# VolkmannB/bayesian-inference-with-explicit-and-implicit-prior-knowledge

Measured on AMD Instinct MI355X. Metric: particle-steps/sec (N x (T-1) / wall), SingleMassOscillator PGAS conditional-SMC sweep, higher is better.
Workload: dtype f64; 1 GPU; SingleMassOscillator PGAS sweep, nx=2, M=41 Hilbert basis (BASELINE.json configs[1]), N=1048576 particles/GPU, T=2000, fp64; particles_per_gpu=1048576, particles_total=1048576, T=2000, partition=single GPU, launch=every sweep enqueued launch by launch, verified=not checked in this run (--full checks the last timed sweep's traces), parallelism=1 GPU

## Files before the change

### bayesian-inference-with-explicit-and-implicit-prior-knowledge_amd/csrc/pgas_api.hip

```cpp
#include <hip/hip_runtime.h>
#include <hip/hip_ext.h>
#include <dlfcn.h>
#include <rccl/rccl.h>

#include <algorithm>
#include <cmath>
#include <cstdio>
#include <cstdlib>
#include <cstring>
#include <string>
#include <vector>

#include "../../include/pgas_hip.h"
#include "pgas_kernels.hip.h"
#include "pgas_resample.hip.h"
#include "pgas_suffstats.hip.h"
#include "pgas_marginal.hip.h"
#include "pgas_marginal_runs.hip.h"
#include "pgas_chains.hip.h"
#include "../../include/pgas_marginal.h"

#ifndef PG_W3
#define PG_W3 2
#endif
// ... 570 lines not shown
    hipLaunchKernelGGL(c->basis, dim3((unsigned)((np + PG_BLK - 1) / PG_BLK)), dim3(PG_BLK), 0, (hipStream_t)stream, c->md, c->d_idx, x_dev, np, t, phi_dev);
    KCHK(c, "k_basis_eval");
    return PGAS_OK;
}

int pgas_aux_states(pgas_ctx* c, const double* x_dev, int32_t t, double* aux_dev, void* stream) {
    if (!c) return PGAS_E_ARG;
    if (!x_dev || !aux_dev || t < 0 || t >= c->md.T) FAIL(c, PGAS_E_ARG, "pgas_aux_states: bad argument");
    if (!c->have_params) FAIL(c, PGAS_E_STATE, "pgas_aux_states: call pgas_set_params first");
    DeviceGuard guard(c->device);
    hipLaunchKernelGGL(c->var.aux, dim3(c->md.nseg), dim3(PG_BLK), 0, (hipStream_t)stream, c->md, (const TransParams*)c->d_tp, t, x_dev, aux_dev);
    KCHK(c, "k_aux");
    return PGAS_OK;
}

int pgas_init_state(pgas_ctx* c, uint64_t seed, const double* ref0_host, double* x0_dev, void* stream) {
    if (!c) return PGAS_E_ARG;
    if (!ref0_host || !x0_dev) FAIL(c, PGAS_E_ARG, "pgas_init_state: NULL argument");
    DeviceGuard guard(c->device);
    hipStream_t st = (hipStream_t)stream;
    HIPCHK(c, hipMemcpyAsync(c->d_ref, ref0_host, c->md.nx * sizeof(double), hipMemcpyHostToDevice, st));
    hipLaunchKernelGGL(c->init, dim3((c->md.N + PG_BLK - 1) / PG_BLK), dim3(PG_BLK), 0, st, c->md, seed, (const SweepParams*)nullptr, c->d_m0L0, c->d_ref, x0_dev);
    KCHK(c, "k_init");
    return PGAS_OK;
}

static Peers peers_for(const pgas_ctx* c, int parity) {
    Peers p = c->peers;
    for (int r = 0; r < p.world; ++r) {
        p.c1[r] = c->peer_c1[parity][r];
        p.c2[r] = c->peer_c2[parity][r];
    }
    return p;
}

static void install_own_peers(pgas_ctx* c) {
    const int r = c->rank;
    for (int k = 0; k < PG_RB_NKIND; ++k) c->peer_blk[r][k].assign(c->rs[k].blk.begin(), c->rs[k].blk.end());
    c->bt_dirty = true;
    for (int i = 0; i < 2; ++i) {
        c->peer_c1[i][r] = c->sb[i].c1;
        c->peer_c2[i][r] = c->sb[i].c2;
    }
}

static const char* peer_row(const pgas_ctx* c, int r, int kind, int t) {
    const RowStore& s = c->rs[kind];
    return c->peer_blk[r][kind][(size_t)t >> s.shift] + (size_t)(t & ((1 << s.shift) - 1)) * s.row_bytes;
}

static int upload_bt_table(pgas_ctx* c, hipStream_t st, BtTab* out) {
    const int nb = std::max(c->rs[PG_RB_X].nblk, c->rs[PG_RB_ANC].nblk);
    const size_t entries = (size_t)c->world * 2 * nb;
    if (c->bt_dirty || c->d_bt_entries != entries) {
        std::vector<const void*> h(entries, nullptr);
        for (int r = 0; r < c->world; ++r) {
            const auto& bx = c->peer_blk[r][PG_RB_X];
            const auto& ba = c->peer_blk[r][PG_RB_ANC];
            for (size_t b = 0; b < bx.size(); ++b) h[((size_t)r * 2) * nb + b] = bx[b];
            for (size_t b = 0; b < ba.size(); ++b) h[((size_t)r * 2 + 1) * nb + b] = ba[b];
        }
        HIPCHK(c, hipStreamSynchronize(st));
        if (c->d_bt_entries != entries) {
            hipFree(c->d_bt);
            c->d_bt = nullptr; c->d_bt_entries = 0;
            HIPCHK(c, hipMalloc(&c->d_bt, entries * sizeof(void*)));
            c->d_bt_entries = entries;
        }
        HIPCHK(c, hipMemcpy(c->d_bt, h.data(), entries * sizeof(void*), hipMemcpyHostToDevice));
        c->bt_dirty = false;
    }
    out->blk = c->d_bt;
    out->nblk_max = nb;
    out->shift_x = c->rs[PG_RB_X].shift;
    out->shift_anc = c->rs[PG_RB_ANC].shift;
    out->entries = (int32_t)entries;
    return PGAS_OK;
}

static int launch_backtrace(pgas_ctx* c, const UpperHdr* hdr, double* traj_dev, hipStream_t st) {
    BtTab tab;
    int rc = upload_bt_table(c, st, &tab);
    if (rc) return rc;
    const size_t lds = tab.entries <= 2048 ? (size_t)tab.entries * sizeof(void*) : 0;
    hipLaunchKernelGGL(k_backtrace, dim3(1), dim3(64), lds, st, c->md.N, c->md.T, c->md.nx, tab, c->world, hdr, traj_dev);
    KCHK(c, "k_backtrace");
    return PGAS_OK;
}

static int launch_groups(pgas_ctx* c, const ScanBufs& sb, int ncdf, hipStream_t st) {
    const int n1 = (c->md.nseg_g + PG_GRP - 1) / PG_GRP;
    hipLaunchKernelGGL(k_groups, dim3((n1 * ncdf + 3) / 4), dim3(256), 0, st, c->md.nseg_g, ncdf, sb);
    KCHK(c, "k_groups");
    return PGAS_OK;
}

static int launch_count(pgas_ctx* c, const ScanBufs& sb, int parity, int what, double u, hipStream_t st) {
    hipLaunchKernelGGL(k_count, dim3(1), dim3(PG_BLK), 0, st, c->md.Ng, c->md.nseg_g, sb, peers_for(c, parity), what, u, what == 1 ? (const SweepParams*)c->d_sp : (const SweepParams*)nullptr);
    KCHK(c, "k_count");
    return PGAS_OK;
}

static bool sweep_is_local(const pgas_ctx* c) { return c->local_groups && c->world == 1 && !c->sharded && c->md.nseg_g <= PG_LOCAL_NSEG && !c->force_slow; }

static bool sweep_tail_groups(const pgas_ctx* c) { return !c->sharded && c->world == 1 && c->tail_groups; }

static int launch_step(pgas_ctx* c, int t, bool local, hipStream_t st, hipEvent_t e0, hipEvent_t e1) {
    const DevModel& md = c->md;
    const int N = md.N, T = md.T;
    StepArgs ar;
    ar.t = t;
    ar.mode = (t < T ? PG_RS_SCAN : 0) | (t > 1 ? PG_RS_SEARCH : 0);
    ar.sp = c->d_sp;
    ar.u_res = c->d_ures;
    ar.u_anc = c->d_uanc;
    ar.la_t = t < T ? (const double*)c->rs[PG_RB_LA].row(t) : (const double*)nullptr;
    ar.h_t = t < T ? (const double*)c->rs[PG_RB_H].row(t) : (const double*)nullptr;
    ar.ln_prev = (const double*)c->rs[PG_RB_LN].row(t - 1);
    ar.anc_in = AncIn{};
    ar.anc_in.has_prev = t > 2 ? 1 : 0;
    if (t > 1)
        for (int r = 0; r < c->world; ++r) {
            ar.anc_in.la_s[r] = (const double*)peer_row(c, r, PG_RB_LA, t - 1);
            ar.anc_in.h_s[r] = (const double*)peer_row(c, r, PG_RB_H, t - 1);
            if (t > 2) {
                ar.anc_in.ln_p[r] = (const double*)peer_row(c, r, PG_RB_LN, t - 2);
                ar.anc_in.la_p[r] = (const double*)peer_row(c, r, PG_RB_LA, t - 2);
                ar.anc_in.anc_p[r] = (const int32_t*)peer_row(c, r, PG_RB_ANC, t - 3);
            }
        }
    ar.anc_out = t > 1 ? (int32_t*)c->rs[PG_RB_ANC].row(t - 2) : (int32_t*)nullptr;
    ar.logw_out = t == T ? c->logw_last : ((c->logw_trace && t > 1) ? c->logw_trace + (size_t)(t - 1) * N : (double*)nullptr);
    const ScanBufs& sp = c->sb[(t - 1) & 1];
    const ScanBufs& sn = c->sb[t & 1];
    const Peers pr = peers_for(c, (t - 1) & 1);
    auto kern = local ? k_step<PG_WM_LOCAL, false> : (sweep_tail_groups(c) ? k_step<PG_WM_GROUPS, true> : k_step<PG_WM_GROUPS, false>);
    if (e0 || e1) hipExtLaunchKernelGGL(kern, dim3(md.nseg + 1), dim3(PG_BLK), 0, st, e0, e1, 0, md, ar, sp, sn, pr);
    else hipLaunchKernelGGL(kern, dim3(md.nseg + 1), dim3(PG_BLK), 0, st, md, ar, sp, sn, pr);
    KCHK(c, "k_step");
    return PGAS_OK;
}

int pgas_step(pgas_ctx* c, int32_t t, uint64_t seed, const double* logw_dev, const double* x_dev, const double* ref_t_host,
              double* logw_new_dev, double* x_new_dev, int32_t* anc_dev, void* stream) {
    if (!c) return PGAS_E_ARG;
    if (!x_dev || !ref_t_host || !logw_new_dev || !x_new_dev || !anc_dev) FAIL(c, PGAS_E_ARG, "pgas_step: NULL argument");
    if (t < 0 || t >= c->md.T) FAIL(c, PGAS_E_ARG, "pgas_step: t = %d outside [0, %d)", t, c->md.T);
    if (!c->have_params) FAIL(c, PGAS_E_STATE, "pgas_step: call pgas_set_params first");
    if (c->sharded) FAIL(c, PGAS_E_STATE, "pgas_step: not available on a shard context");
    DeviceGuard guard(c->device);
    hipStream_t st = (hipStream_t)stream;
    const DevModel& md = c->md;
    install_own_peers(c);
    HIPCHK(c, hipMemcpyAsync(c->d_ref, ref_t_host, md.nx * sizeof(double), hipMemcpyHostToDevice, st));
    if (c->corrected && !c->aux_buf) HIPCHK(c, hipMalloc(&c->aux_buf, (size_t)md.N * md.nx * sizeof(double)));
    hipLaunchKernelGGL(c->var.front, dim3(md.nseg), dim3(PG_BLK), 0, st, md, (const TransParams*)c->d_tp, t, seed, x_dev, logw_dev, c->d_ref, c->corrected,
                       c->corrected ? c->aux_buf : x_new_dev, c->sb[0]);
    KCHK(c, "k_front");
    int rc = launch_groups(c, c->sb[0], 2, st);
    if (rc) return rc;
    rc = launch_count(c, c->sb[0], 0, 0, pgas_rng_uniform(seed, PGAS_STREAM_ANCESTOR, (uint32_t)t), st);
    if (rc) return rc;
    const Peers pr = peers_for(c, 0);
    if (c->corrected) {
        hipLaunchKernelGGL(c->back_corrected, dim3(md.nseg), dim3(PG_BLK), 0, st, md, (const TransParams*)c->d_tp, t, seed,
                           pgas_rng_uniform(seed, PGAS_STREAM_RESAMPLE, (uint32_t)t), c->aux_buf, c->d_ref, c->sb[0], pr, anc_dev, x_new_dev, logw_new_dev);
    } else {
        hipLaunchKernelGGL(c->back, dim3(md.nseg), dim3(PG_BLK), 0, st, md, t,
// ... 493 lines not shown
    }
    FAIL(c, PGAS_E_ARG, "pgas_set_option: unknown option %d", option);
}

int pgas_get_profile(pgas_ctx* c, int64_t* launches, double* total_ms, int64_t* propagate_launches, double* propagate_ms, void* stream) {
    if (!c) return PGAS_E_ARG;
    if (!launches || !total_ms || !propagate_launches || !propagate_ms) FAIL(c, PGAS_E_ARG, "pgas_get_profile: NULL argument");
    DeviceGuard guard(c->device);
    HIPCHK(c, hipStreamSynchronize((hipStream_t)stream));
    double sum = 0.0;
    for (int i = 0; i + 1 < c->ev_used; i += 2) {
        float ms = 0.f;
        HIPCHK(c, hipEventElapsedTime(&ms, c->ev[i], c->ev[i + 1]));
        sum += ms;
    }
    *launches = c->ev_used / 2;
    *total_ms = sum;
    double psum = 0.0;
    for (int i = 0; i + 1 < c->evp_used; i += 2) {
        float ms = 0.f;
        HIPCHK(c, hipEventElapsedTime(&ms, c->evp[i], c->evp[i + 1]));
        psum += ms;
    }
    *propagate_launches = c->evp_used / 2;
    *propagate_ms = psum;
    return PGAS_OK;
}

int pgas_get_launch_info(pgas_ctx* c, int32_t* info4) {
    if (!c) return PGAS_E_ARG;
    if (!info4) FAIL(c, PGAS_E_ARG, "pgas_get_launch_info: NULL argument");
    info4[0] = c->last_chunk;
    info4[1] = (c->last_small ? 3 : (sweep_is_local(c) ? 1 : (sweep_tail_groups(c) ? 2 : 0))) + (c->last_graph ? 16 : 0) + ((c->d_mxi && c->use_mx && !c->last_small) ? 32 : 0);
    info4[2] = c->md.JP;
    info4[3] = c->var_P;
    return PGAS_OK;
}

#ifdef PG_DEBUG_DUMP
int pgas_debug_dump(double* out ) {
    return hipMemcpyFromSymbol(out, HIP_SYMBOL(g_dbg), sizeof(double) * 4 * 64) == hipSuccess ? 0 : -2;
}
#endif
#ifdef PG_STAMPS
int pgas_debug_stamps(unsigned long long* out ) {
    return hipMemcpyFromSymbol(out, HIP_SYMBOL(g_stamps), sizeof(unsigned long long) * 2048 * 16) == hipSuccess ? 0 : -2;
}
#endif


static int systematic_impl(pgas_ctx* c, double u, const double* u_dev, const double* logw_dev, int32_t* idx_dev, void* stream) {
    if (c->sharded) FAIL(c, PGAS_E_STATE, "pgas_systematic_resample: not available on a shard context");
    DeviceGuard guard(c->device);
    hipStream_t st = (hipStream_t)stream;
    const DevModel& md = c->md;
    install_own_peers(c);
    hipLaunchKernelGGL(k_segscan, dim3(md.nseg), dim3(PG_BLK), 0, st, md.N, logw_dev, c->sb[0]);
    KCHK(c, "k_segscan");
    int rc = launch_groups(c, c->sb[0], 1, st);
    if (rc) return rc;
    hipLaunchKernelGGL(k_systematic, dim3(md.nseg), dim3(PG_BLK), 0, st, md, u, u_dev, c->sb[0], peers_for(c, 0), idx_dev);
    KCHK(c, "k_systematic");
    return PGAS_OK;
}

int pgas_systematic_resample(pgas_ctx* c, double u, const double* logw_dev, int32_t* idx_dev, void* stream) {
    if (!c) return PGAS_E_ARG;
    if (!logw_dev || !idx_dev || !(u >= 0.0 && u < 1.0)) FAIL(c, PGAS_E_ARG, "pgas_systematic_resample: bad argument");
    return systematic_impl(c, u, nullptr, logw_dev, idx_dev, stream);
}

int pgas_systematic_resample_dev(pgas_ctx* c, const double* u_dev, const double* logw_dev, int32_t* idx_dev, void* stream) {
    if (!c) return PGAS_E_ARG;
    if (!u_dev || !logw_dev || !idx_dev) FAIL(c, PGAS_E_ARG, "pgas_systematic_resample_dev: NULL argument");
    return systematic_impl(c, 0.0, u_dev, logw_dev, idx_dev, stream);
}

int pgas_reconstruct_trajectory(pgas_ctx* c, const double* x_dev, const int32_t* anc_dev, int32_t T, int32_t nx, int64_t idx,
                                double* traj_dev, void* stream) {
    if (!c) return PGAS_E_ARG;
    if (!x_dev || !traj_dev || T < 1 || nx < 1 || idx < 0 || idx >= c->md.N || (T > 1 && !anc_dev))
        FAIL(c, PGAS_E_ARG, "pgas_reconstruct_trajectory: bad argument");
    DeviceGuard guard(c->device);
    hipLaunchKernelGGL(k_backtrace_idx, dim3(1), dim3(64), 0, (hipStream_t)stream, c->md.N, T, nx, x_dev, anc_dev, idx, traj_dev);
    KCHK(c, "k_backtrace_idx");
    return PGAS_OK;
}

int pgas_shard_setup(pgas_ctx* c, int32_t rank, int32_t world) {
    if (!c) return PGAS_E_ARG;
    if (world < 1 || world > PG_MAX_RANKS || rank < 0 || rank >= world) FAIL(c, PGAS_E_ARG, "pgas_shard_setup: bad rank/world %d/%d", rank, world);
    if (c->md.N % PGAS_SEG) FAIL(c, PGAS_E_ARG, "pgas_shard_setup: local particle count %d must be a multiple of %d", c->md.N, PGAS_SEG);
    if ((int64_t)c->md.nseg * world > PG_MAX_NSEG) FAIL(c, PGAS_E_ARG, "pgas_shard_setup: %d global segments exceed %d", c->md.nseg * world, PG_MAX_NSEG);
    if (c->sharded) FAIL(c, PGAS_E_STATE, "pgas_shard_setup: already set up");
    if (c->corrected) FAIL(c, PGAS_E_STATE, "pgas_shard_setup: the corrected mode is not available on a sharded context");
    DeviceGuard guard(c->device);
    if (c->have_traces && c->rs[PG_RB_X].contiguous) {
        HIPCHK(c, hipDeviceSynchronize());
        for (RowStore& r : c->rs) r.release();
        hipFree(c->logw_last); hipFree(c->logw_trace);
        c->logw_last = c->logw_trace = nullptr;
        c->have_traces = false;
    }
    int rc = ensure_traces(c, true);
    if (rc) return rc;
    const int nsegp = c->sb[0].nsegp, nseg_g = c->md.nseg * world, nsegp_g = (nseg_g + 63) / 64 * 64;
    double* segk_g[2] = {nullptr, nullptr};
    uint64_t* segs_g[2] = {nullptr, nullptr};
    double* tab[2][3] = {{nullptr, nullptr, nullptr}, {nullptr, nullptr, nullptr}};
    hipError_t e = hipSuccess;
    for (int i = 0; i < 2 && e == hipSuccess; ++i) {
        e = hipMalloc(&segk_g[i], (size_t)world * 2 * nsegp * sizeof(double));
        if (e == hipSuccess) e = hipMalloc(&segs_g[i], (size_t)world * 2 * nsegp * sizeof(uint64_t));
        for (int k = 0; k < 3 && e == hipSuccess; ++k) e = hipMalloc(&tab[i][k], 2 * (size_t)nsegp_g * sizeof(double));
        if (e == hipSuccess) e = hipMemset(segk_g[i], 0, (size_t)world * 2 * nsegp * sizeof(double));
        if (e == hipSuccess) e = hipMemset(segs_g[i], 0, (size_t)world * 2 * nsegp * sizeof(uint64_t));
    }
    if (e != hipSuccess) {
        for (int i = 0; i < 2; ++i) {
            hipFree(segk_g[i]); hipFree(segs_g[i]);
            for (int k = 0; k < 3; ++k) hipFree(tab[i][k]);
        }
        FAIL(c, e == hipErrorOutOfMemory ? PGAS_E_NOMEM : PGAS_E_HIP, "pgas_shard_setup: allocation failed: %s", hipGetErrorString(e));
    }
    DevModel& md = c->md;
    c->rank = rank; c->world = world;
    md.p0 = (int64_t)rank * md.N;
    md.Ng = md.N * world;
    md.nseg_g = nseg_g;
    for (int r = 0; r < PG_MAX_RANKS; ++r) {
        for (int k = 0; k < PG_RB_NKIND; ++k) c->peer_blk[r][k].clear();
        c->peer_c1[0][r] = c->peer_c1[1][r] = c->peer_c2[0][r] = c->peer_c2[1][r] = nullptr;
    }
    c->peers.world = world; c->peers.nseg_l = md.nseg; c->peers.Nl = md.N;
    for (int i = 0; i < 2; ++i) {
        ScanBufs& sb = c->sb[i];
        c->segk_g[i] = segk_g[i]; c->segs_g[i] = segs_g[i];
        sb.segk = segk_g[i]; sb.segs = segs_g[i];
        sb.nseg_l = md.nseg; sb.rank_stride = 2 * nsegp; sb.nsegp_g = nsegp_g;
        hipFree(sb.tab_e); hipFree(sb.tab_sc); hipFree(sb.tab_m);
        sb.tab_e = tab[i][0]; sb.tab_sc = tab[i][1]; sb.tab_m = tab[i][2];
    }
    c->sharded = true;
    install_own_peers(c);
    return PGAS_OK;
}

int pgas_shard_buffers(pgas_ctx* c, void** out, int64_t* sizes) {
    if (!c) return PGAS_E_ARG;
    if (!c->sharded) FAIL(c, PGAS_E_STATE, "pgas_shard_buffers: call pgas_shard_setup first");
    if (!out || !sizes) FAIL(c, PGAS_E_ARG, "pgas_shard_buffers: NULL argument");
    out[0] = c->sb[0].c1; out[1] = c->sb[1].c1;
    out[2] = c->rs[PG_RB_LA].blk[0]; out[3] = c->rs[PG_RB_H].blk[0]; out[4] = c->rs[PG_RB_LN].blk[0]; out[5] = c->rs[PG_RB_X].blk[0]; out[6] = c->rs[PG_RB_ANC].blk[0];
    out[7] = c->sb[0].c2; out[8] = c->sb[1].c2;
    out[9] = c->sb[0].segk_w; out[10] = c->sb[1].segk_w; out[11] = c->sb[0].segs_w; out[12] = c->sb[1].segs_w;
    out[13] = c->segk_g[0]; out[14] = c->segk_g[1]; out[15] = c->segs_g[0]; out[16] = c->segs_g[1];
    sizes[0] = c->sb[0].nsegp; sizes[1] = c->md.N; sizes[2] = c->md.T;
    return PGAS_OK;
}

static int shard_which_kind(int which) {
    static const int k[7] = {-1, -1, PG_RB_LA, PG_RB_H, PG_RB_LN, PG_RB_X, PG_RB_ANC};
    return k[which];
}

int pgas_shard_layout(pgas_ctx* c, int32_t which, int64_t* info2) {
    if (!c) return PGAS_E_ARG;
// ... 827 lines not shown
```

### bayesian-inference-with-explicit-and-implicit-prior-knowledge_amd/csrc/pgas_kernels.hip.h

```cpp
#pragma once

#include <hip/hip_runtime.h>
#include <stdint.h>

#include "../../include/pgas_canon.h"

#define PG_BLK 256
#define PG_PPT 4
static_assert(PG_BLK * PG_PPT == PGAS_SEG && PGAS_SEG == 1024, "one workgroup owns one canonical segment of 1024 particles");
#define PG_UPPER_THREADS 256
#define PG_MAX_NSEG 8192

#ifdef PG_STAMPS
__device__ unsigned long long g_stamps[2048 * 16];
#define PG_STAMP(id)                                                                                \
    do {                                                                                            \
        if (threadIdx.x == 0) g_stamps[blockIdx.x * 16 + (id)] = __builtin_amdgcn_s_memrealtime(); \
    } while (0)
#else
#define PG_STAMP(id) do { } while (0)
#endif


#ifndef PG_NO_STREAM_STORES
// ... 1066 lines not shown
            }
#pragma unroll kUnroll
            for (int r0 = 0; r0 < PPT; r0 += P) {
                if (seg0 + r0 / PG_PPT >= md.nseg) break;
                double xin[P][NX], xn[P][NX], la[P], h[P], ln[P];
#pragma unroll
                for (int p = 0; p < P; ++p) {
#pragma unroll
                    for (int k = 0; k < NX; ++k) xin[p][k] = ONE ? xnext[p][k] : xv[ONE ? 0 : r0 + p][k];
                }
                if constexpr (ONE) {
                    const int rn = r0 + P < PPT ? r0 + P : r0;
#pragma unroll
                    for (int p = 0; p < P; ++p) load_state(rn + p, xnext[p]);
                }
                if constexpr (MX) {
                    double aux[P][NX];
                    eval_mean_mx<NX, JIN, MXD>(md, Guse, mx_tab, ut, xin[0], aux[0]);
                    propagate_finish<NX, P>(md, tp, t, seed, rf, yt, seg0 + r0 / PG_PPT, r0 % PG_PPT, aux, xn, la, h, ln);
                } else {
                    propagate_group<NX, D, JIN, P, J0T>(md, tp, Guse, t, seed, rf, yt, ut, seg0 + r0 / PG_PPT, r0 % PG_PPT, xin, xn, la, h, ln);
                }
#pragma unroll
                for (int p = 0; p < P; ++p) {
                    const size_t pi = particle(r0 + p);
                    if (pi < (size_t)md.N) {
                        if constexpr (NX == 2) {
#ifdef PG_NT_X
                            typedef double pg_d2 __attribute__((ext_vector_type(2)));
                            pg_d2 v2 = {xn[p][0], xn[p][1]};
                            __builtin_nontemporal_store(v2, reinterpret_cast<pg_d2*>(xt) + pi);
#else
                            reinterpret_cast<double2*>(xt)[pi] = make_double2(xn[p][0], xn[p][1]);
#endif
                        } else {
#pragma unroll
                            for (int k = 0; k < NX; ++k) xt[pi * NX + k] = xn[p][k];
                        }
                    }
#ifdef PG_NT_H
                    __builtin_nontemporal_store(la[p], &la_rows[hrow + pi]);
                    __builtin_nontemporal_store(h[p], &h_rows[hrow + pi]);
                    __builtin_nontemporal_store(ln[p], &ln_rows[hrow + pi]);
#else
                    la_rows[hrow + pi] = la[p];
                    h_rows[hrow + pi] = h[p];
                    ln_rows[hrow + pi] = ln[p];
#endif
                    if constexpr (!ONE) {
#pragma unroll
                        for (int k = 0; k < NX; ++k) xv[r0 + p][k] = xn[p][k];
                    }
                }
            }
        }
    }
}

template <int NX, int D, int JIN, int P, int W, int J0T = 0, int PPT = PG_PPT, bool ONE = false>
__global__ __launch_bounds__(PG_BLK, W) void k_propagate(DevModel md, const TransParams* __restrict__ tpp, const double* __restrict__ G, const SweepParams* __restrict__ swp, int t0, int t1,
                                                          const double* __restrict__ x_prev, double* __restrict__ x_rows, const double* __restrict__ ref,
                                                          double* __restrict__ la_rows, double* __restrict__ h_rows, double* __restrict__ ln_rows) {
    propagate_kernel<NX, D, JIN, P, J0T, PPT, ONE>(md, tpp, G, swp, t0, t1, x_prev, x_rows, ref, la_rows, h_rows, ln_rows);
}
template <int NX, int JIN, int W, int PPT, bool ONE, uint64_t MXD>
__global__ __launch_bounds__(PG_BLK, W) void k_propagate_mx(DevModel md, const TransParams* __restrict__ tpp, const double* __restrict__ G, const SweepParams* __restrict__ swp, int t0, int t1,
                                                             const double* __restrict__ x_prev, double* __restrict__ x_rows, const double* __restrict__ ref,
                                                             double* __restrict__ la_rows, double* __restrict__ h_rows, double* __restrict__ ln_rows,
                                                             const MxInfo* __restrict__ mxi, const double* __restrict__ gimg) {
    propagate_kernel<NX, 3, JIN, 1, 0, PPT, ONE, MXD>(md, tpp, G, swp, t0, t1, x_prev, x_rows, ref, la_rows, h_rows, ln_rows, mxi, gimg);
}
__global__ __launch_bounds__(PG_BLK) void k_segscan(int N, const double* __restrict__ logw, ScanBufs sb) {
    __shared__ ScanSmem sm;
    const int seg = blockIdx.x, tid = threadIdx.x;
    double lw[1][PG_PPT];
#pragma unroll
    for (int r = 0; r < PG_PPT; ++r) {
        const int64_t i = (int64_t)seg * PGAS_SEG + r * PG_BLK + tid;
        lw[0][r] = i < N ? logw[i] : -__builtin_inf();
    }
    segment_scan<1>(sm, lw, seg, sb.nsegp, sb.c1, nullptr, sb.segk_w, sb.segs_w);
}

__global__ void k_backtrace(int Nl, int T, int nx, BtTab tab, int world, const UpperHdr* __restrict__ hdr, double* __restrict__ traj) {
    extern __shared__ const void* pg_bt_lds[];
    const bool in_lds = tab.entries <= 2048;
    if (in_lds) {
        for (int i = threadIdx.x; i < tab.entries; i += blockDim.x) pg_bt_lds[i] = tab.blk[i];
        __syncthreads();
    }
    if (threadIdx.x != 0 || blockIdx.x != 0) return;
    const void* const* blk = in_lds ? pg_bt_lds : tab.blk;
    const int mx = (1 << tab.shift_x) - 1, ma = (1 << tab.shift_anc) - 1;
    int64_t b = hdr->final_idx;
    for (int i = T - 1; i >= 0; --i) {
        const int r = world > 1 ? (int)(b / Nl) : 0;
        const int64_t bl = b - (int64_t)r * Nl;
        const double* __restrict__ xr = (const double*)blk[(size_t)(r * 2) * tab.nblk_max + (i >> tab.shift_x)] + (size_t)(i & mx) * Nl * nx;
        for (int k = 0; k < nx; ++k) traj[(size_t)i * nx + k] = xr[(size_t)bl * nx + k];
        if (i > 0) {
            const int32_t* __restrict__ ar = (const int32_t*)blk[(size_t)(r * 2 + 1) * tab.nblk_max + ((i - 1) >> tab.shift_anc)] + (size_t)((i - 1) & ma) * Nl;
            b = ar[bl];
        }
    }
}

template <int NX>
__global__ __launch_bounds__(PG_BLK) void k_basis_eval(DevModel md, const int32_t* __restrict__ idx, const double* __restrict__ x,
                                                        int64_t np, int t, double* __restrict__ phi) {
    const int64_t p = (int64_t)blockIdx.x * PG_BLK + threadIdx.x;
    if (p >= np) return;
    const double* __restrict__ ut = md.u + (size_t)t * md.nu;
    double xv[NX];
#pragma unroll
    for (int k = 0; k < NX; ++k) xv[k] = x[p * NX + k];
    double sv[PGAS_MAX_D][PGAS_MAX_J];
    for (int d = 0; d < md.D; ++d) dim_sines_point<NX>(md, d, xv, ut, sv[d]);
    for (int m = 0; m < md.M; ++m) {
        double f = md.nrm;
        for (int d = 0; d < md.D; ++d) f = f * sv[d][(idx[m * md.D + d] - md.j0[d]) / md.jstep[d]];
        phi[p * md.M + m] = f;
    }
}

template <int NX, int D, int JIN, int P>
__global__ __launch_bounds__(PG_BLK) void k_aux(DevModel md, const TransParams* __restrict__ tpp, int t, const double* __restrict__ x, double* __restrict__ aux_out) {
    const int seg = blockIdx.x, tid = threadIdx.x;
    const TransParams tp = *tpp;
    double xv[PG_PPT][NX];
    load_particles<NX>(md, x, seg, xv);
    const double* __restrict__ ut = md.u + (size_t)t * md.nu;
#pragma unroll
    for (int r0 = 0; r0 < PG_PPT; r0 += P) {
        double xin[P][NX], aux[P][NX];
#pragma unroll
        for (int p = 0; p < P; ++p)
#pragma unroll
            for (int k = 0; k < NX; ++k) xin[p][k] = xv[r0 + p][k];
        eval_mean<NX, D, JIN, P>(md, tp.G, ut, xin, aux);
#pragma unroll
        for (int p = 0; p < P; ++p) {
            const int64_t pi = (int64_t)seg * PGAS_SEG + (r0 + p) * PG_BLK + tid;
            if (pi < md.N)
#pragma unroll
                for (int k = 0; k < NX; ++k) aux_out[pi * NX + k] = aux[p][k];
        }
    }
}
```

### bayesian-inference-with-explicit-and-implicit-prior-knowledge_amd/csrc/pgas_resample.hip.h

```cpp
#pragma once

#include "pgas_kernels.hip.h"

#define PG_GRP PGAS_GRP
#define PG_MAX_GRP (PG_MAX_NSEG / PG_GRP)
#define PG_WIN_SEG 1024
#define PG_WIN_GRP (PG_WIN_SEG / PG_GRP)
#define PG_LOCAL_NSEG PG_WIN_SEG
#ifndef PG_FSTAGE
#define PG_FSTAGE 2
#endif
#define PG_NCAND 8
#define PG_DEXP_ZERO (-32768)
#ifdef PG_COLD_NOINLINE
#define PG_COLD_ATTR __noinline__
#else
#define PG_COLD_ATTR __forceinline__
#endif
static_assert(PG_MAX_GRP <= 128, "top_scan_wave handles two blocks of 64 groups");
#ifdef PG_DEBUG_DUMP
__device__ double g_dbg[4][64];
#endif

__device__ __forceinline__ size_t partial_at(const ScanBufs& sb, int cdf, int b) {
// ... 645 lines not shown
    const double* __restrict__ yt = md.y + (size_t)t * md.ny;
    double z0[PG_PPT], z1[PG_PPT];
    {
        pgas_u32x4 w[PG_PPT];
#pragma unroll
        for (int r = 0; r < PG_PPT; ++r) {
            const int64_t pi = (int64_t)seg * PGAS_SEG + r * PG_BLK + tid;
            w[r] = pgas_rng_block(seed, PGAS_STREAM_PROP, 0u, (uint32_t)t, (uint64_t)(md.p0 + pi));
        }
        pgas_normal_pair_n(w, z0, z1, PG_PPT);
    }
    double xn[PG_PPT][NX];
#pragma unroll
    for (int r = 0; r < PG_PPT; ++r) {
        const int64_t pi = (int64_t)seg * PGAS_SEG + r * PG_BLK + tid;
        const int src = pi < md.N ? anc[r] : 0;
        const double z[2] = {z0[r], z1[r]};
#pragma unroll
        for (int k = 0; k < NX; ++k) {
            double v = aux[(size_t)src * NX + k];
#pragma unroll
            for (int l = 0; l <= k; ++l) v = PGAS_FMA(tp.LS[k * NX + l], z[l], v);
            xn[r][k] = (md.p0 + pi == md.Ng - 1) ? ref_t[k] : v;
        }
        if (pi < md.N) logw_out[pi] = loglik<NX>(md, yt, xn[r]) - sb.laux[src];
    }
    store_particles<NX>(md, x_new, seg, xn);
}

__global__ __launch_bounds__(PG_BLK) void k_systematic(DevModel md, double u, const double* __restrict__ u_dev, ScanBufs sb, Peers pr,
                                                      int32_t* __restrict__ idx_out) {
    __shared__ WinSmemT<PG_WM_GROUPS> sm;
    int anc[PG_PPT];
    resample_slots<PG_WM_GROUPS>(md, sm, u_dev ? u_dev[0] : u, sb, pr, blockIdx.x, idx_out, anc, -1);
}

#define PG_RS_SEARCH 1
#define PG_RS_SCAN 2

struct StepArgs {
    int t, mode;
    const SweepParams* sp;
    const double* u_res;
    const double* u_anc;
    const double* la_t;
    const double* h_t;
    const double* ln_prev;
    AncIn anc_in;
    int32_t* anc_out;
    double* logw_out;
};

template <int LOCAL>
__device__ PG_COLD_ATTR int cdf_count_wg_cold(WinSmemT<LOCAL>& sm, const ScanBufs& sb, const Peers& pr, int nseg, int N, double U, const AncIn& in) {
    return cdf_count_wg<LOCAL>(sm, sb, pr, 1, nseg, N, U, nullptr, nullptr, &in);
}

#ifndef PG_STEP_OCC
#define PG_STEP_OCC 4
#endif
template <int LOCAL, bool TAIL = false>
__global__ __launch_bounds__(PG_BLK, PG_STEP_OCC) void k_step(DevModel md, StepArgs ar, ScanBufs sb_prev, ScanBufs sb_next, Peers pr) {
    __shared__ WinSmemT<LOCAL> sm;
    const int tid = threadIdx.x;
    const int N = md.N;
    const unsigned tag = ar.sp->epoch * 2654435761u + (unsigned)ar.t;
    const double u1_prev = (ar.mode & PG_RS_SEARCH) ? ar.u_res[ar.t - 1] : 0.0, u2_prev = (ar.mode & PG_RS_SEARCH) ? ar.u_anc[ar.t - 1] : 0.0;
#ifdef PG_STEP_PRIO
    __builtin_amdgcn_s_setprio(PG_STEP_PRIO);
#endif
    if (blockIdx.x == 0) {
        if (!(ar.mode & PG_RS_SEARCH)) return;
        const int r = cdf_count_wg<LOCAL>(sm, sb_prev, pr, 1, md.nseg_g, md.Ng, u2_prev, nullptr, nullptr, &ar.anc_in);
        if (tid == 0)
            __hip_atomic_store(&sb_prev.hdr->ref_granule, ((unsigned long long)tag << 32) | (unsigned)r, __ATOMIC_RELAXED,
                               __HIP_MEMORY_SCOPE_AGENT);
        return;
    }
    const int seg = blockIdx.x - 1;
    const int64_t base_i = (int64_t)seg * PGAS_SEG;
    PG_STAMP(0);
    double lnv[PG_PPT] = {0.0, 0.0, 0.0, 0.0};
    double lwp[PG_PPT] = {0.0, 0.0, 0.0, 0.0};
    if (ar.mode & PG_RS_SEARCH) {
        int a[PG_PPT];
        resample_search<LOCAL>(md, sm, u1_prev, sb_prev, pr, seg, a, [&]() {
#pragma unroll
            for (int r = 0; r < PG_PPT; ++r) lnv[r] = ld_stream(&ar.ln_prev[(size_t)base_i + r * PG_BLK + tid]);
        });
        const bool last_wg = md.p0 + base_i + PGAS_SEG >= md.Ng;
        if (last_wg) {
            __syncthreads();
            if (tid == 0) {
                unsigned long long g = 0;
                int spins = 0;
                for (; spins < (1 << 16); ++spins) {
                    g = __hip_atomic_load(&sb_prev.hdr->ref_granule, __ATOMIC_RELAXED, __HIP_MEMORY_SCOPE_AGENT);
                    if ((unsigned)(g >> 32) == tag) break;
                    __builtin_amdgcn_s_sleep(8);
                }
                sm.cnt[1] = ((unsigned)(g >> 32) == tag) ? (int)(unsigned)g : -1;
            }
            __syncthreads();
            int ref_idx = sm.cnt[1];
            if (ref_idx < 0) {
                __syncthreads();
                ref_idx = cdf_count_wg_cold<LOCAL>(sm, sb_prev, pr, md.nseg_g, md.Ng, u2_prev, ar.anc_in);
            }
#pragma unroll
            for (int j = 0; j < PG_PPT; ++j)
                if (md.p0 + base_i + slot_of(tid, j) == md.Ng - 1) a[j] = ref_idx;
        }
        PG_STAMP(4);
        __syncthreads();
#pragma unroll
        for (int j = 0; j < PG_PPT; ++j) {
            sm.u.a[slot_of(tid, j)] = a[j];
            if (base_i + slot_of(tid, j) < N) st_stream(&ar.anc_out[base_i + slot_of(tid, j)], (int32_t)a[j]);
        }
        __syncthreads();
        int anv[PG_PPT];
        double lav[PG_PPT];
#pragma unroll
        for (int r = 0; r < PG_PPT; ++r) anv[r] = sm.u.a[r * PG_BLK + tid];
        if (pr.world == 1) {
            const double* __restrict__ la0 = ar.anc_in.la_s[0];
#pragma unroll
            for (int r = 0; r < PG_PPT; ++r) lav[r] = la0[anv[r]];
        } else {
            const double* rowp[PG_PPT];
            int off[PG_PPT];
#pragma unroll
            for (int r = 0; r < PG_PPT; ++r) {
                const int ra = anv[r] / pr.Nl;
                off[r] = anv[r] - ra * pr.Nl;
                rowp[r] = ar.anc_in.la_s[ra];
            }
#pragma unroll
            for (int r = 0; r < PG_PPT; ++r) lav[r] = rowp[r][off[r]];
        }
#pragma unroll
        for (int r = 0; r < PG_PPT; ++r) {
            const int64_t i = base_i + r * PG_BLK + tid;
            lwp[r] = i < N ? lnv[r] - lav[r] : 0.0;
        }
        PG_STAMP(5);
        if (ar.logw_out != nullptr) {
#pragma unroll
            for (int r = 0; r < PG_PPT; ++r) {
                const int64_t i = base_i + r * PG_BLK + tid;
                if (i < N) ar.logw_out[i] = lwp[r];
            }
        }
        __syncthreads();
    }
    if (ar.mode & PG_RS_SCAN) {
        double lw[2][PG_PPT];
        {
            double lat[PG_PPT], ht[PG_PPT];
#pragma unroll
            for (int r = 0; r < PG_PPT; ++r) {
                const size_t pi = (size_t)base_i + r * PG_BLK + tid;
                lat[r] = ld_stream(&ar.la_t[pi]);
                ht[r] = ld_stream(&ar.h_t[pi]);
            }
#pragma unroll
            for (int r = 0; r < PG_PPT; ++r) {
                const size_t pi = (size_t)base_i + r * PG_BLK + tid;
                const bool valid_p = pi < (size_t)N;
                const double l1 = lat[r] + lwp[r];
                lw[0][r] = valid_p ? l1 : -__builtin_inf();
                lw[1][r] = valid_p ? l1 + ht[r] : -__builtin_inf();
            }
        }
        PG_STAMP(6);
        segment_scan<2, false, TAIL>(sm.u.scan, lw, seg, sb_next.nsegp, sb_next.c1, sb_next.c2, sb_next.segk_w, sb_next.segs_w);
        PG_STAMP(8);
        if constexpr (TAIL) {
            if (tid < 64) {
                const int g = seg / PG_GRP;
                const int nb = md.nseg - g * PG_GRP < PG_GRP ? md.nseg - g * PG_GRP : PG_GRP;
                unsigned arrived = 0;
                if (tid == 0) {
                    asm volatile("s_waitcnt vmcnt(0)" ::: "memory");
                    arrived = __hip_atomic_fetch_add(&sb_next.grp_cnt[g], 1u, __ATOMIC_RELAXED, __HIP_MEMORY_SCOPE_AGENT);
                }
                arrived = __builtin_amdgcn_readfirstlane(arrived);
                if (arrived == (unsigned)(nb - 1)) {
                    __builtin_amdgcn_fence(__ATOMIC_ACQUIRE, "agent");
                    asm volatile("s_waitcnt vmcnt(0)" ::: "memory");
                    group_records_wave(sb_next, md.nseg, 0, g, true);
                    group_records_wave(sb_next, md.nseg, 1, g, true);
                    if (tid == 0) __hip_atomic_store(&sb_next.grp_cnt[g], 0u, __ATOMIC_RELAXED, __HIP_MEMORY_SCOPE_AGENT);
                }
            }
        }
    }
    PG_STAMP(7);
}

__global__ void k_backtrace_idx(int N, int T, int nx, const double* __restrict__ x_trace, const int32_t* __restrict__ anc_trace,
                                int64_t idx, double* __restrict__ traj) {
    if (threadIdx.x != 0 || blockIdx.x != 0) return;
    int64_t b = idx;
    for (int i = T - 1; i >= 0; --i) {
        for (int k = 0; k < nx; ++k) traj[(size_t)i * nx + k] = x_trace[((size_t)i * N + b) * nx + k];
        if (i > 0) b = anc_trace[(size_t)(i - 1) * N + b];
    }
}

__global__ void k_detmath(int which, const double* __restrict__ x, const double* __restrict__ y, const uint32_t* __restrict__ w,
                          int64_t n, double* __restrict__ o0, double* __restrict__ o1, uint32_t* __restrict__ ow) {
    const int64_t i = (int64_t)blockIdx.x * blockDim.x + threadIdx.x;
    if (i >= n) return;
    switch (which) {
    case 0: o0[i] = pgas_exp(x[i]); break;
    case 1: o0[i] = pgas_log(x[i]); break;
    case 2: pgas_sincospi(x[i], &o0[i], &o1[i]); break;
    case 3: {
        const pgas_u32x4 r = pgas_philox4x32_10(w[6 * i], w[6 * i + 1], w[6 * i + 2], w[6 * i + 3], w[6 * i + 4], w[6 * i + 5]);
        for (int k = 0; k < 4; ++k) ow[4 * i + k] = r.v[k];
        break;
    }
    case 4: o0[i] = pgas_seg_ref(x[i]); break;
    case 5: o0[i] = pgas_seg_arg(x[i], y[i]); break;
    case 6: o0[i] = pgas_lvl_scale(x[i], y[i]); break;
    case 7: {
        const pgas_u32x4 r = pgas_philox4x32_10(w[6 * i], w[6 * i + 1], w[6 * i + 2], w[6 * i + 3], w[6 * i + 4], w[6 * i + 5]);
        pgas_normal_pair(r, &o0[i], &o1[i]);
        break;
    }
    case 8: {
        const double xv[1] = {x[i]};
        uint64_t qv[1];
        dev_exp_q51_n<1>(xv, qv);
        o0[i] = (double)qv[0];
        break;
    }
    default: break;
    }
}

__device__ __forceinline__ void lds_barrier() { asm volatile("s_waitcnt lgkmcnt(0)\n\ts_barrier" ::: "memory"); }

__global__ __launch_bounds__(256) void k_small_noise(const SweepParams* __restrict__ swp, int64_t p0, int N, int T, double* __restrict__ znoise) {
    const int64_t q = (int64_t)blockIdx.x * 256 + threadIdx.x;
    if (q >= (int64_t)N * (T - 1)) return;
    const int t = 1 + (int)(q / N), i = (int)(q % N);
    double z0, z1;
    pgas_normal_pair(pgas_rng_block(ld_const(&swp->seed), PGAS_STREAM_PROP, 0u, (uint32_t)t, (uint64_t)(p0 + i)), &z0, &z1);
    znoise[((size_t)t * N + i) * 2] = z0;
    znoise[((size_t)t * N + i) * 2 + 1] = z1;
}

template <int NX, int D, int JIN, int J0T>
__device__ __forceinline__ void small_particle_step(const DevModel& md, const TransParams& tp, const double* __restrict__ G, const double* __restrict__ ut,
                                                    const double* __restrict__ yt, const double (&rf)[NX], bool conditioned, const double (&xin)[1][NX],
                                                    const double (&z)[2], double (&xt)[NX], double& la, double& h, double& ln) {
    double aux[1][NX];
    eval_mean<NX, D, JIN, 1, J0T, true>(md, G, ut, xin, aux);
    la = loglik<NX>(md, yt, aux[0]);
    double quad = 0.0;
#pragma unroll
    for (int k = 0; k < NX; ++k) {
        double w = 0.0;
#pragma unroll
        for (int l = 0; l <= k; ++l) w = PGAS_FMA(tp.LSinv[k * NX + l], rf[l] - aux[0][l], w);
        quad = PGAS_FMA(w, w, quad);
    }
    h = PGAS_FMA(-0.5, quad, tp.cS);
#pragma unroll
    for (int k = 0; k < NX; ++k) {
        double v = aux[0][k];
#pragma unroll
        for (int l = 0; l <= k; ++l) v = PGAS_FMA(tp.LS[k * NX + l], z[l], v);
        xt[k] = conditioned ? rf[k] : v;
    }
    ln = loglik<NX>(md, yt, xt);
}

struct SmallSmem {
    uint64_t q[2][PGAS_SEG];
    double num[2][PGAS_SEG];
    double la[PGAS_SEG];
    double red[2][PG_BLK / 64];
    uint64_t wtot[2][PG_BLK / 64];
    int cnt[PG_BLK / 64];
};

template <int NW, int NR>
__device__ __forceinline__ void small_scan(SmallSmem& sm, const double (&lw)[NW][NR], int n, double (&S)[NW]) {
// ... 515 lines not shown
```

Before: 33.40 billion particle-steps/s.

## Split backtrace into serial ancestor chase and parallel trajectory gather

The backtrace kernel now has one thread chase the ancestor chain in chunks, recording indices to LDS. All 256 threads then gather the state rows in parallel, using vectorized 2-double loads when nx==2. It is templated on multi-rank so the single-GPU path drops the per-step division, and it prefetches the next ancestor row pointer. The resample kernel also moves its ancestor trace store to the end of the kernel, taking it off the path before the LDS exchange. The serial dependent-load chain remains, so gains are bounded by latency.

```diff
diff --git a/bayesian-inference-with-explicit-and-implicit-prior-knowledge_amd/csrc/pgas_api.hip b/bayesian-inference-with-explicit-and-implicit-prior-knowledge_amd/csrc/pgas_api.hip
--- a/bayesian-inference-with-explicit-and-implicit-prior-knowledge_amd/csrc/pgas_api.hip
+++ b/bayesian-inference-with-explicit-and-implicit-prior-knowledge_amd/csrc/pgas_api.hip
@@ -676,8 +676,9 @@
     BtTab tab;
     int rc = upload_bt_table(c, st, &tab);
     if (rc) return rc;
-    const size_t lds = tab.entries <= 2048 ? (size_t)tab.entries * sizeof(void*) : 0;
-    hipLaunchKernelGGL(k_backtrace, dim3(1), dim3(64), lds, st, c->md.N, c->md.T, c->md.nx, tab, c->world, hdr, traj_dev);
+    const size_t lds = tab.entries <= PG_BT_TAB_LDS ? (size_t)tab.entries * sizeof(void*) : 0;
+    if (c->world > 1) hipLaunchKernelGGL(k_backtrace<true>, dim3(1), dim3(PG_BT_THREADS), lds, st, c->md.N, c->md.T, c->md.nx, tab, hdr, traj_dev);
+    else hipLaunchKernelGGL(k_backtrace<false>, dim3(1), dim3(PG_BT_THREADS), lds, st, c->md.N, c->md.T, c->md.nx, tab, hdr, traj_dev);
     KCHK(c, "k_backtrace");
     return PGAS_OK;
 }
@@ -1337,7 +1338,7 @@
     if (!x_dev || !traj_dev || T < 1 || nx < 1 || idx < 0 || idx >= c->md.N || (T > 1 && !anc_dev))
         FAIL(c, PGAS_E_ARG, "pgas_reconstruct_trajectory: bad argument");
     DeviceGuard guard(c->device);
-    hipLaunchKernelGGL(k_backtrace_idx, dim3(1), dim3(64), 0, (hipStream_t)stream, c->md.N, T, nx, x_dev, anc_dev, idx, traj_dev);
+    hipLaunchKernelGGL(k_backtrace_idx, dim3(1), dim3(PG_BT_THREADS), 0, (hipStream_t)stream, c->md.N, T, nx, x_dev, anc_dev, idx, traj_dev);
     KCHK(c, "k_backtrace_idx");
     return PGAS_OK;
 }
diff --git a/bayesian-inference-with-explicit-and-implicit-prior-knowledge_amd/csrc/pgas_kernels.hip.h b/bayesian-inference-with-explicit-and-implicit-prior-knowledge_amd/csrc/pgas_kernels.hip.h
--- a/bayesian-inference-with-explicit-and-implicit-prior-knowledge_amd/csrc/pgas_kernels.hip.h
+++ b/bayesian-inference-with-explicit-and-implicit-prior-knowledge_amd/csrc/pgas_kernels.hip.h
@@ -1172,27 +1172,98 @@
     segment_scan<1>(sm, lw, seg, sb.nsegp, sb.c1, nullptr, sb.segk_w, sb.segs_w);
 }
 
-__global__ void k_backtrace(int Nl, int T, int nx, BtTab tab, int world, const UpperHdr* __restrict__ hdr, double* __restrict__ traj) {
+#define PG_BT_THREADS 256
+#define PG_BT_CHUNK 4096
+#define PG_BT_TAB_LDS 2048
+#define PG_GLOBAL_AS __attribute__((address_space(1)))
+typedef const PG_GLOBAL_AS int32_t* pg_gi32p;
+typedef const PG_GLOBAL_AS double* pg_gf64p;
+typedef const void* pg_cvoidp;
+
+struct BtTabLds {
+    __device__ __forceinline__ const void* operator[](uint32_t k) const {
+        extern __shared__ const void* pg_bt_lds[];
+        return pg_bt_lds[k];
+    }
+};
+struct BtTabGlobal {
+    const PG_GLOBAL_AS pg_cvoidp* p;
+    __device__ __forceinline__ const void* operator[](uint32_t k) const { return p[k]; }
+};
+
+template <class AncRowFn>
+__device__ __forceinline__ uint32_t bt_chase_rows(int hi, int lo, uint32_t b, int32_t* rec, AncRowFn anc_row) {
+    pg_gi32p nxt = anc_row(hi > 0 ? hi - 1 : 0);
+    for (int i = hi; i >= lo; --i) {
+        rec[i - lo] = (int32_t)b;
+        if (i == 0) break;
+        const pg_gi32p cur = nxt;
+        nxt = anc_row(i > 1 ? i - 2 : 0);
+        b = (uint32_t)cur[b];
+    }
+    return b;
+}
+
+template <class ChaseFn, class XAtFn>
+__device__ __forceinline__ void bt_passes(int T, int nx, uint32_t b, int32_t* rec, double* __restrict__ traj, bool vec2, ChaseFn chase, XAtFn x_at) {
+    for (int hi = T - 1; hi >= 0; hi -= PG_BT_CHUNK) {
+        const int lo = hi >= PG_BT_CHUNK ? hi - PG_BT_CHUNK + 1 : 0;
+        if (threadIdx.x == 0) b = chase(hi, lo, b, rec);
+        __syncthreads();
+        for (int i = lo + (int)threadIdx.x; i <= hi; i += PG_BT_THREADS) {
+            const pg_gf64p xp = x_at(i, (uint32_t)rec[i - lo]);
+            if (vec2) {
+                *(pg_nt_d2*)&traj[(size_t)i * 2] = *(const PG_GLOBAL_AS pg_nt_d2*)xp;
+            } else {
+                for (int k = 0; k < nx; ++k) traj[(size_t)i * nx + k] = xp[k];
+            }
+        }
+        if (lo > 0) __syncthreads();
+    }
+}
+
+template <bool MULTI, class Tab>
+__device__ __forceinline__ void bt_sweep(int Nl, int T, int nx, const BtTab& tab, Tab blk, uint32_t b, int32_t* rec, double* __restrict__ traj) {
+    const int sx = tab.shift_x, sa = tab.shift_anc, mx = (1 << sx) - 1, ma = (1 << sa) - 1;
+    const uint32_t nb = (uint32_t)tab.nblk_max;
+    const bool vec2 = nx == 2 && ((uintptr_t)traj & 15) == 0;
+    if constexpr (!MULTI) {
+        auto anc_row = [&](int i) { return (pg_gi32p)blk[nb + (uint32_t)(i >> sa)] + (size_t)(i & ma) * Nl; };
+        bt_passes(T, nx, b, rec, traj, vec2,
+                  [&](int hi, int lo, uint32_t bb, int32_t* rc) { return bt_chase_rows(hi, lo, bb, rc, anc_row); },
+                  [&](int i, uint32_t bi) { return (pg_gf64p)blk[(uint32_t)(i >> sx)] + ((size_t)(i & mx) * Nl + bi) * nx; });
+    } else {
+        const uint32_t nl = (uint32_t)Nl;
+        bt_passes(T, nx, b, rec, traj, vec2,
+                  [&](int hi, int lo, uint32_t bb, int32_t* rc) {
+                      for (int i = hi; i >= lo; --i) {
+                          rc[i - lo] = (int32_t)bb;
+                          if (i == 0) break;
+                          const uint32_t r = bb / nl, bl = bb - r * nl;
+                          const pg_gi32p ar = (pg_gi32p)blk[(r * 2 + 1) * nb + (uint32_t)((i - 1) >> sa)] + (size_t)((i - 1) & ma) * Nl;
+                          bb = (uint32_t)ar[bl];
+                      }
+                      return bb;
+                  },
+                  [&](int i, uint32_t bi) {
+                      const uint32_t r = bi / nl, bl = bi - r * nl;
+                      return (pg_gf64p)blk[(r * 2) * nb + (uint32_t)(i >> sx)] + ((size_t)(i & mx) * Nl + bl) * nx;
+                  });
+    }
+}
+
+template <bool MULTI>
+__global__ __launch_bounds__(PG_BT_THREADS) void k_backtrace(int Nl, int T, int nx, BtTab tab, const UpperHdr* __restrict__ hdr, double* __restrict__ traj) {
     extern __shared__ const void* pg_bt_lds[];
-    const bool in_lds = tab.entries <= 2048;
+    __shared__ int32_t rec[PG_BT_CHUNK];
+    const bool in_lds = tab.entries <= PG_BT_TAB_LDS;
     if (in_lds) {
-        for (int i = threadIdx.x; i < tab.entries; i += blockDim.x) pg_bt_lds[i] = tab.blk[i];
+        for (int i = threadIdx.x; i < tab.entries; i += PG_BT_THREADS) pg_bt_lds[i] = tab.blk[i];
         __syncthreads();
     }
-    if (threadIdx.x != 0 || blockIdx.x != 0) return;
-    const void* const* blk = in_lds ? pg_bt_lds : tab.blk;
-    const int mx = (1 << tab.shift_x) - 1, ma = (1 << tab.shift_anc) - 1;
-    int64_t b = hdr->final_idx;
-    for (int i = T - 1; i >= 0; --i) {
-        const int r = world > 1 ? (int)(b / Nl) : 0;
-        const int64_t bl = b - (int64_t)r * Nl;
-        const double* __restrict__ xr = (const double*)blk[(size_t)(r * 2) * tab.nblk_max + (i >> tab.shift_x)] + (size_t)(i & mx) * Nl * nx;
-        for (int k = 0; k < nx; ++k) traj[(size_t)i * nx + k] = xr[(size_t)bl * nx + k];
-        if (i > 0) {
-            const int32_t* __restrict__ ar = (const int32_t*)blk[(size_t)(r * 2 + 1) * tab.nblk_max + ((i - 1) >> tab.shift_anc)] + (size_t)((i - 1) & ma) * Nl;
-            b = ar[bl];
-        }
-    }
+    const uint32_t b = threadIdx.x == 0 ? (uint32_t)hdr->final_idx : 0u;
+    if (in_lds) bt_sweep<MULTI>(Nl, T, nx, tab, BtTabLds{}, b, rec, traj);
+    else bt_sweep<MULTI>(Nl, T, nx, tab, BtTabGlobal{(const PG_GLOBAL_AS pg_cvoidp*)tab.blk}, b, rec, traj);
 }
 
 template <int NX>
diff --git a/bayesian-inference-with-explicit-and-implicit-prior-knowledge_amd/csrc/pgas_resample.hip.h b/bayesian-inference-with-explicit-and-implicit-prior-knowledge_amd/csrc/pgas_resample.hip.h
--- a/bayesian-inference-with-explicit-and-implicit-prior-knowledge_amd/csrc/pgas_resample.hip.h
+++ b/bayesian-inference-with-explicit-and-implicit-prior-knowledge_amd/csrc/pgas_resample.hip.h
@@ -751,8 +751,13 @@
     PG_STAMP(0);
     double lnv[PG_PPT] = {0.0, 0.0, 0.0, 0.0};
     double lwp[PG_PPT] = {0.0, 0.0, 0.0, 0.0};
+    int a[PG_PPT] = {0, 0, 0, 0};
+    auto store_trace = [&]() {
+#pragma unroll
+        for (int j = 0; j < PG_PPT; ++j)
+            if (base_i + slot_of(tid, j) < N) st_stream(&ar.anc_out[base_i + slot_of(tid, j)], (int32_t)a[j]);
+    };
     if (ar.mode & PG_RS_SEARCH) {
-        int a[PG_PPT];
         resample_search<LOCAL>(md, sm, u1_prev, sb_prev, pr, seg, a, [&]() {
 #pragma unroll
             for (int r = 0; r < PG_PPT; ++r) lnv[r] = ld_stream(&ar.ln_prev[(size_t)base_i + r * PG_BLK + tid]);
@@ -783,10 +788,7 @@
         PG_STAMP(4);
         __syncthreads();
 #pragma unroll
-        for (int j = 0; j < PG_PPT; ++j) {
-            sm.u.a[slot_of(tid, j)] = a[j];
-            if (base_i + slot_of(tid, j) < N) st_stream(&ar.anc_out[base_i + slot_of(tid, j)], (int32_t)a[j]);
-        }
+        for (int j = 0; j < PG_PPT; ++j) sm.u.a[slot_of(tid, j)] = a[j];
         __syncthreads();
         int anv[PG_PPT];
         double lav[PG_PPT];
@@ -865,17 +867,20 @@
             }
         }
     }
+    if (ar.mode & PG_RS_SEARCH) store_trace();
     PG_STAMP(7);
 }
 
-__global__ void k_backtrace_idx(int N, int T, int nx, const double* __restrict__ x_trace, const int32_t* __restrict__ anc_trace,
-                                int64_t idx, double* __restrict__ traj) {
-    if (threadIdx.x != 0 || blockIdx.x != 0) return;
-    int64_t b = idx;
-    for (int i = T - 1; i >= 0; --i) {
-        for (int k = 0; k < nx; ++k) traj[(size_t)i * nx + k] = x_trace[((size_t)i * N + b) * nx + k];
-        if (i > 0) b = anc_trace[(size_t)(i - 1) * N + b];
-    }
+__global__ __launch_bounds__(PG_BT_THREADS) void k_backtrace_idx(int N, int T, int nx, const double* __restrict__ x_trace, const int32_t* __restrict__ anc_trace,
+                                                                 int64_t idx, double* __restrict__ traj) {
+    __shared__ int32_t rec[PG_BT_CHUNK];
+    const pg_gi32p anc = (pg_gi32p)anc_trace;
+    const pg_gf64p x = (pg_gf64p)x_trace;
+    const bool vec2 = nx == 2 && (((uintptr_t)traj | (uintptr_t)x_trace) & 15) == 0;
+    auto anc_row = [&](int i) { return anc + (size_t)i * N; };
+    bt_passes(T, nx, (uint32_t)idx, rec, traj, vec2,
+              [&](int hi, int lo, uint32_t b, int32_t* rc) { return bt_chase_rows(hi, lo, b, rc, anc_row); },
+              [&](int i, uint32_t b) { return x + ((size_t)i * N + b) * nx; });
 }
 
 __global__ void k_detmath(int which, const double* __restrict__ x, const double* __restrict__ y, const uint32_t* __restrict__ w,
```

New measurement: 34.83 billion particle-steps/s, median of 6. 4.3% higher.
